# kirumang/Pix2Pose

Hardware: AMD Instinct MI355X
Metric: crops/sec (AE fwd + PnP-RANSAC) at 128x128 (higher is better)
Workload: dtype f16x3 (fp32 operands split into two f16 halves, 3 MFMAs per product block, fp32 accumulate)

## Files before the change

### include/p2p_mi355.h

```cpp
#ifndef P2P_MI355_H
#define P2P_MI355_H

#include <stdint.h>

#ifdef __cplusplus
extern "C" {
#endif

#define P2P_ABI_VERSION 12

#if defined(__GNUC__)
#define P2P_API __attribute__((visibility("default")))
#else
#define P2P_API
#endif

typedef enum {
    P2P_OK = 0,
    P2P_ERR_INVALID_ARG = -1,
    P2P_ERR_HIP = -2,
    P2P_ERR_WEIGHTS = -3,
    P2P_ERR_CAPACITY = -4,
    P2P_ERR_RANGE = -5
} p2p_status;
// ... 5 lines not shown
typedef struct p2p_ctx p2p_ctx;
typedef struct p2p_model p2p_model;

typedef struct {
    const char* name;
    const float* data;
    int64_t numel;
} p2p_tensor;

P2P_API int p2p_abi_version(void);
P2P_API int p2p_abi_sizeof(int which);
P2P_API const char* p2p_build_id(void);
P2P_API int p2p_aa_weights(int side, double* w);
P2P_API int p2p_debug_back_resize(p2p_ctx* ctx, const float* prob, const float* pred, const float* non_gray, int out_h, int out_w,
                                  double th_inlier, int generation, unsigned char* q, unsigned char* below, unsigned char* ng_out);
P2P_API const char* p2p_last_error(void);
P2P_API int p2p_device_count(int* count);

P2P_API int p2p_ctx_create(int device, int max_batch, p2p_ctx** out);
P2P_API void p2p_ctx_destroy(p2p_ctx* ctx);
P2P_API int p2p_ctx_synchronize(p2p_ctx* ctx);
P2P_API void* p2p_ctx_stream(p2p_ctx* ctx);

P2P_API int p2p_model_create(p2p_ctx* ctx, const p2p_tensor* tensors, int n_tensors, int backbone,
                     p2p_model** out);

typedef enum { P2P_PREC_F32 = 0, P2P_PREC_F16X3 = 1, P2P_PREC_AUTO = 2 } p2p_precision;
#define P2P_PREC_DEFAULT P2P_PREC_F16X3
P2P_API int p2p_model_create_ex(p2p_ctx* ctx, const p2p_tensor* tensors, int n_tensors, int backbone,
                        int precision, p2p_model** out);
// ... 296 lines not shown
```

### pix2pose_amd/_lib.py

```python
from __future__ import annotations

import ctypes as C
import os

_HERE = os.path.dirname(os.path.abspath(__file__))
LIB_PATH = os.environ.get("P2P_LIB", os.path.join(_HERE, "libp2p_mi355.so"))

P2P_OK = 0
ABI_VERSION = 12
MAX_RANSAC_ITERATIONS = 128
BACKBONE = {"paper": 0, "resnet50": 1}
PRECISION = {"f32": 0, "f16x3": 1, "auto": 2}
ERR_RANGE = -5
MEM_HOST, MEM_DEVICE = 0, 1
COMM_ID_BYTES = 128
POSE_ABSENT = -1
POSE_RANGE = -2
TICKET_NONE = -1


class P2PError(RuntimeError):
    pass


# ... 213 lines not shown
        except Exception as e:
            raise P2PError("libp2p_mi355.so is %s and could not be rebuilt: %s" % (reason, e))
        reason = _stale_reason(LIB_PATH)
        if reason is not None:
            raise P2PError("%s: %s after a rebuild" % (LIB_PATH, reason))
    _preload_torch_hip()
    try:
        L = C.CDLL(LIB_PATH)
    except OSError as e:
        raise P2PError("cannot load %s: %s (the HIP path is mandatory, there is no fallback)" % (LIB_PATH, e))
    vp, fp, ci = C.c_void_p, C.POINTER(C.c_float), C.c_int
    L.p2p_abi_version.restype = ci
    L.p2p_abi_sizeof.argtypes = [ci]
    L.p2p_build_id.restype = C.c_char_p
    L.p2p_aa_weights.argtypes = [ci, C.POINTER(C.c_double)]
    L.p2p_last_error.restype = C.c_char_p
    L.p2p_device_count.argtypes = [C.POINTER(ci)]
    L.p2p_ctx_create.argtypes = [ci, ci, C.POINTER(vp)]
    L.p2p_ctx_destroy.argtypes = [vp]
    L.p2p_ctx_destroy.restype = None
    L.p2p_ctx_synchronize.argtypes = [vp]
    L.p2p_ctx_stream.argtypes = [vp]
    L.p2p_ctx_stream.restype = vp
    L.p2p_model_create.argtypes = [vp, C.POINTER(Tensor), ci, ci, C.POINTER(vp)]
    L.p2p_model_create_ex.argtypes = [vp, C.POINTER(Tensor), ci, ci, ci, C.POINTER(vp)]
    L.p2p_model_destroy.argtypes = [vp]
    L.p2p_model_destroy.restype = None
    L.p2p_model_precision.argtypes = [vp]
    L.p2p_ctx_range_event.argtypes = [vp, C.POINTER(C.c_float)]
    L.p2p_ctx_set_winograd.argtypes = [vp, ci]
# ... 56 lines not shown
```

### pix2pose_amd/csrc/kernels.h

```cpp
#pragma once
#include <hip/hip_runtime.h>
#include <stdint.h>
#include <stdlib.h>

namespace p2p {

#ifdef P2P_DEV_SWITCHES
inline const char* dev_env(const char* name) { return getenv(name); }
#else
inline const char* dev_env(const char*) { return nullptr; }
#endif

struct Ctx;
extern thread_local Ctx* g_prof_ctx;
struct ProfScope {
    Ctx* ctx;
    hipStream_t s;
    int slot;
    double flops, bytes;
    hipEvent_t a = nullptr, b = nullptr;
    bool failed = false;
    ProfScope(Ctx* X, int slot_, hipStream_t st, double fl = 0.0, double by = 0.0) : ctx(X), s(st), slot(slot_), flops(fl), bytes(by) { if (ctx) open(); }
    ProfScope(int slot_, hipStream_t st) : ProfScope(g_prof_ctx, slot_, st) {}
    ~ProfScope() { if (ctx) (void)close(); }
// ... 89 lines not shown

int igemm_halo8_mode(const IgemmParams& p);
hipError_t launch_igemm_halo8(const IgemmParams& p, hipStream_t s);

bool igemm_halo_s2_supported(const IgemmParams& p);
hipError_t launch_igemm_halo_s2(const IgemmParams& p, hipStream_t s);

struct ResBlockGroup {
    const float* w2a;
    const float* w2b;
    const float* w2c;
    const float* ss;
    int sample0;
    int pad_;
    const float* w2b_frag;
};
struct ResBlockParams {
    const float* x;
    float* out;
    int N, H, W;
    unsigned x_bytes, wa_bytes, wb_bytes, wc_bytes;
    unsigned* range_acc;
    int n_groups;
    ResBlockGroup grp[IGEMM_MAX_GROUPS + 1];
};
bool resblock_supported(int F1, int H, int W);
int resblock_grid(int F1, int N, int H, int W);
hipError_t launch_resblock(const ResBlockParams& p, int F1, hipStream_t s);
hipError_t launch_resproj(const ResBlockParams& p, int F1, hipStream_t s);

struct WinoGroup {
// ... 131 lines not shown
```

### pix2pose_amd/csrc/model.hip

```cpp
#include "model.h"

#include <cmath>
#include <cstdarg>
#include <cstdio>
#include <cstring>
#include <thread>

namespace p2p {

static thread_local char g_err[512] = "";

void set_error(const char* fmt, ...)
{
    va_list ap;
    va_start(ap, fmt);
    vsnprintf(g_err, sizeof(g_err), fmt, ap);
    va_end(ap);
}
const char* get_error() { return g_err; }

constexpr double BN_EPS = 1e-3;
constexpr float LEAKY = 0.3f;

struct TensorMap {
// ... 604 lines not shown
        if ((rc = pack_wino3_s2(T, {"conv4_1", "conv4_2"}, 512, 256, M.L["conv4"]))) return rc;
        return build_decoder(T, M, 128, 128, 32);
    }
    if (M.backbone == P2P_BACKBONE_PAPER) {
        if ((rc = pack_conv_first(T, {"conv1_1", "conv1_2"}, 5, 64, M.L["conv1"]))) return rc;
        if ((rc = pack_conv(T, {"conv2_1", "conv2_2"}, 5, 128, 128, 1, true, M.L["conv2"]))) return rc;
        if ((rc = pack_conv(T, {"conv3_1", "conv3_2"}, 5, 256, 128, 1, true, M.L["conv3"]))) return rc;
        if ((rc = pack_conv(T, {"conv4_1", "conv4_2"}, 5, 256, 256, 1, true, M.L["conv4"]))) return rc;
        if ((rc = pack_wino3_s2(T, {"conv4_1", "conv4_2"}, 256, 256, M.L["conv4"]))) return rc;
        return build_decoder(T, M, 128, 128, 64);
    }
    set_error("unknown backbone %d", M.backbone);
    return P2P_ERR_INVALID_ARG;
}

static int pack_block_ss(Model& M)
{
    if (M.backbone != P2P_BACKBONE_RESNET50 || M.prec != PREC_F16X3) return P2P_OK;
    for (const char* nm : {"res2a", "res2b", "res2c", "res3a", "res3b", "res3c", "res3d"}) {
        const std::string n = nm;
        if (!M.L.count(n + "_2c") && !M.L.count(n + "_2c1")) continue;
        const ConvLayer &a = M.L.at(n + "_2a"), &b = M.L.at(n + "_2b"), &c = M.L.count(n + "_2c") ? M.L.at(n + "_2c") : M.L.at(n + "_2c1");
        const int F1 = a.Cout, C = c.Cout;
        float* d = nullptr;
        HIP_TRY(hipMalloc((void**)&d, (size_t)(4 * F1 + 2 * C) * sizeof(float)));
        M.block_ss[n] = d;
        if (!M.L.at(n + "_2b").w_frag) {
            ConvLayer& Lb = M.L.at(n + "_2b");
            const int K = Lb.K, KS = K / 32, NTL = Lb.Cout / 32;
            std::vector<float> host((size_t)round_up(Lb.Cout, 128) * K), frag((size_t)Lb.Cout * K);
            HIP_TRY(hipMemcpy(host.data(), Lb.w, host.size() * sizeof(float), hipMemcpyDeviceToHost));
            const uint16_t* sh = reinterpret_cast<const uint16_t*>(host.data());
            uint16_t* dh = reinterpret_cast<uint16_t*>(frag.data());
            for (int nt = 0; nt < NTL; ++nt)
                for (int ks = 0; ks < KS; ++ks)
                    for (int f = 0; f < 4; ++f)
                        for (int lane = 0; lane < 64; ++lane) {
                            const int row = nt * 32 + (lane & 31), kb = f >> 1, hf = f & 1;
                            const uint16_t* sp = sh + ((size_t)row * K + (size_t)ks * 32) * 2 + hf * 32 + kb * 16 + (lane >> 5) * 8;
                            uint16_t* dp = dh + ((((size_t)nt * KS + ks) * 4 + f) * 64 + lane) * 8;
                            for (int e = 0; e < 8; ++e) dp[e] = sp[e];
                        }
            int rcu = upload(frag, &Lb.w_frag);
            if (rcu) return rcu;
        }
        const float* src[6] = {a.scale, a.shift, b.scale, b.shift, c.scale, c.shift};
        const int len[6] = {F1, F1, F1, F1, C, C};
        size_t off = 0;
        for (int k = 0; k < 6; ++k) {
            HIP_TRY(hipMemcpy(d + off, src[k], (size_t)len[k] * sizeof(float), hipMemcpyDeviceToDevice));
            off += len[k];
        }
    }
    return P2P_OK;
}

constexpr size_t WINO_PARTIAL_FLOATS = (size_t)256 * 16 * 32 * 64;
static const struct { const char* name; size_t per_sample; } kBuffers[] = {
// ... 481 lines not shown
    const size_t xb = (size_t)N * H * H * Cin * sizeof(float), ob = (size_t)N * Ho * Ho * C * sizeof(float);
    if (xb >= 0xFFFFFFF0ull || ob >= 0xFFFFFFF0ull) { set_error("run_fused_block: tensor exceeds the 4 GB buffer-descriptor range (lower max_batch)"); return P2P_ERR_CAPACITY; }
    p.x_bytes = (unsigned)xb;
    p.wa_bytes = (unsigned)((size_t)round_up(a.Cout, 128) * a.K * sizeof(float));
    p.wb_bytes = (unsigned)((size_t)round_up(b.Cout, 128) * b.K * sizeof(float));
    p.wc_bytes = (unsigned)((size_t)round_up(c.Cout, 128) * c.K * sizeof(float));
    p.range_acc = X.range_cur;
    const int ng = pass_groups(X, "run_fused_block");
    if (ng < 0) return ng;
    if (ng) {
        const GroupCtx& G = *X.grp;
        for (int g = 0; g < ng; ++g) {
            const Model& Mg = *G.models[g];
            const ConvLayer* bg = group_layer(X, g, b, false);
            if (!bg || !Mg.block_ss.count(n)) return group_mismatch("run_fused_block");
            p.grp[g] = {Mg.L.at(a.name).w, bg->w, Mg.L.at(c.name).w, Mg.block_ss.at(n), G.start[g], 0, bg->w_frag};
        }
        p.grp[ng] = {nullptr, nullptr, nullptr, nullptr, G.start[ng], 0, nullptr};
        p.n_groups = ng;
    } else {
        p.grp[0] = {a.w, b.w, c.w, M.block_ss.at(n), 0, 0, b.w_frag};
        p.grp[1] = {nullptr, nullptr, nullptr, nullptr, N, 0, nullptr};
        p.n_groups = 1;
    }
    const double px = (double)N * Ho * Ho;
    return prof_launch(X, 9, 2.0 * px * ((double)Cin * f1 + 9.0 * f1 * f1 + (double)c.K * C),
                       4.0 * (px * Cin + px * C + (double)Cin * f1 + 9.0 * f1 * f1 + (double)c.K * C),
                       [&]() { return proj ? launch_resproj(p, f1, X.cur->stream) : launch_resblock(p, f1, X.cur->stream); });
}

static bool fused_proj_blocks() { static const bool on = dev_env("P2P_NO_FUSED_PROJ") == nullptr; return on; }

static int res_block(const Model& M, Ctx& X, const std::string& n, const float* in, int N, int H,
                     int Cin, int f1, int stride, bool shortcut, float* out)
{
    int rc;
    const int Ho = H / stride;
// ... 287 lines not shown
    case 3: return (int)sizeof(p2p_detection);
    case 4: return (int)sizeof(p2p_pose);
    case 5: return (int)sizeof(p2p_est_pose_opts);
    case 6: return (int)sizeof(p2p_kernel_stats);
    case 7: return (int)sizeof(p2p_refine_job);
    case 8: return (int)sizeof(p2p_depth_score);
    case 9: return (int)sizeof(p2p_icp_input);
    case 10: return (int)sizeof(p2p_icp_params);
    case 11: return (int)sizeof(p2p_icp_result);
    case 12: return (int)sizeof(p2p_refine_result);
    default: return -1;
    }
}
const char* p2p_last_error(void) { return get_error(); }

int p2p_device_count(int* count)
{
    if (!count) { set_error("p2p_device_count: null argument"); return P2P_ERR_INVALID_ARG; }
    HIP_TRY(hipGetDeviceCount(count));
    return P2P_OK;
}

int p2p_ctx_create(int device, int max_batch, p2p_ctx** out)
{
    if (!out || max_batch < 1) { set_error("p2p_ctx_create: bad arguments"); return P2P_ERR_INVALID_ARG; }
    *out = nullptr;
    int n = 0;
    HIP_TRY(hipGetDeviceCount(&n));
    if (device < 0 || device >= n) { set_error("p2p_ctx_create: device %d out of range (%d devices)", device, n); return P2P_ERR_INVALID_ARG; }
    HIP_TRY(hipSetDevice(device));
// ... 189 lines not shown
```

### pix2pose_amd/csrc/resblock.hip

```cpp
#include "device_common.h"

namespace p2p {

namespace {

constexpr int REC = 144;
constexpr int WREC = 128;

constexpr int cmax(int a, int b) { return a > b ? a : b; }

#ifdef P2P_RB_NO_WDIR
constexpr bool RB_WDIR = false;
#else
constexpr bool RB_WDIR = true;
#endif
#ifndef P2P_RB_DA64
#define P2P_RB_DA64 2
#endif
#ifndef P2P_RB_DA3A
#define P2P_RB_DA3A 2
#endif
#ifdef P2P_RB_NO_PIPE
constexpr bool RB_PIPE = false;
#else
constexpr bool RB_PIPE = true;
#endif
#ifdef P2P_RB_NO_DBUF
constexpr bool RB_DBUF = false;
#else
constexpr bool RB_DBUF = true;
#endif
template <int F1, int PY, int HPX, int DA, int DB, int KA, bool PRIV, int ABL = 0, int CIN = 4 * F1, int STRIDE = 1, bool PROJ = false, bool WDIR = RB_WDIR, bool DBUF = RB_DBUF, bool PIPE = RB_PIPE>
__global__ __launch_bounds__(256, 2) void resblock_kernel(const ResBlockParams p)
{
    constexpr int C = 4 * F1;
    constexpr int SA = CIN / 32;
    constexpr int SX = CIN / 32;
    static_assert(PROJ || (CIN == C && STRIDE == 1), "identity blocks keep their shape");
    constexpr int SB = F1 / 32;
    constexpr int NCH = C / 128;
    constexpr int HX0 = HPX == 18 ? 1 : 0;
    constexpr int HPY = PY + 2, NPA = HPY * HPX, MA = (NPA + 31) / 32;
    constexpr int PITCH = (HPX * REC + 255) / 256 * 256;
    constexpr int TSLICE = HPY * PITCH, T_BYTES = SB * TSLICE;
    constexpr int NPIX = PY * 16, MT = PY / 2;
    constexpr int T2SLICE = NPIX * REC, T2_BYTES = SB * T2SLICE;
    constexpr int XS_BYTES = MA * 32 * REC;
    constexpr int WA_BYTES = F1 * WREC;
    constexpr int WB_BYTES = PRIV ? 4 * 32 * WREC : F1 * WREC;
    constexpr int WC_BYTES = 2 * 128 * WREC;
    constexpr int NST = SB / 2;
    constexpr int TMC = 2, TNC = MT == 4 ? 2 : 1, WGMC = MT / TMC, WGNC = 4 / WGMC;
    constexpr int CLD = 128 + 4;
    constexpr int CS_BYTES = TMC * 32 * CLD * 4;
    constexpr int XC_BYTES = NPIX * REC;
    constexpr int NBUF = DBUF ? 2 : KA;
    static_assert(!DBUF || (KA == 1 && DA % 2 == 0), "double buffering: one K-step per stage, buffer parity = ring slot parity");
    constexpr int ZERO_OFF = cmax(cmax(NBUF * (XS_BYTES + WA_BYTES), T_BYTES + WB_BYTES),
                                  T2_BYTES + cmax(PROJ ? 128 * WREC + XC_BYTES : WC_BYTES, CS_BYTES));
    constexpr int SS_OFF = ZERO_OFF + 128, SS_FLOATS = 4 * F1 + 2 * C;
    constexpr int SMEM = SS_OFF + SS_FLOATS * 4;
    static_assert(SMEM <= 80 * 1024, "two workgroups per CU");
    static_assert(MA % (F1 == 64 ? 2 : 1) == 0 && (F1 == 64 || F1 == 128) && (PY == 8 || PY == 4), "shapes");
    __shared__ __attribute__((aligned(256))) char smem[SMEM];
    static_assert(SS_FLOATS % 4 == 0, "float4 copies");

    const int tid = threadIdx.x;
    const int lane = tid & 63, wave = __builtin_amdgcn_readfirstlane(tid >> 6);
    const int li = lane & 31, lk = lane >> 5;

    const int tiles_x = p.W / 16, tiles_y = p.H / PY;
    int t = xcd_first_tile(gridDim.x, blockIdx.x);
    const int x0 = (t % tiles_x) * 16; t /= tiles_x;
    const int y0 = (t % tiles_y) * PY;
    const int n = t / tiles_y;

    int g = 0;
    while (g + 1 < p.n_groups && p.grp[g + 1].sample0 <= n) ++g;
    const float* ss = reinterpret_cast<const float*>(smem + SS_OFF);
    for (int i = tid * 4; i < SS_FLOATS; i += 1024)
        *reinterpret_cast<f32x4*>(smem + SS_OFF + i * 4) = *reinterpret_cast<const f32x4*>(p.grp[g].ss + i);
    const __amdgpu_buffer_rsrc_t rs_x = __builtin_amdgcn_make_buffer_rsrc((void*)p.x, 0, p.x_bytes, 0x00020000);
    const __amdgpu_buffer_rsrc_t rs_wa = __builtin_amdgcn_make_buffer_rsrc((void*)p.grp[g].w2a, 0, p.wa_bytes, 0x00020000);
    const __amdgpu_buffer_rsrc_t rs_wb = __builtin_amdgcn_make_buffer_rsrc((void*)p.grp[g].w2b, 0, p.wb_bytes, 0x00020000);
    const __amdgpu_buffer_rsrc_t rs_wc = __builtin_amdgcn_make_buffer_rsrc((void*)p.grp[g].w2c, 0, p.wc_bytes, 0x00020000);

    if (tid < 8) *reinterpret_cast<f32x4*>(smem + ZERO_OFF + tid * 16) = f32x4{0.f, 0.f, 0.f, 0.f};

    const int lrow = tid >> 3, lseg = tid & 7;
    const int w_dst = lrow * WREC + ((lseg ^ ((lrow >> 1) & 7)) << 4);
    float amax = 0.f;

    f32x16 accA[3];
#pragma unroll
    for (int i = 0; i < 3; ++i)
#pragma unroll
        for (int r = 0; r < 16; ++r) accA[i][r] = 0.f;
    constexpr int WNA = F1 / 32 >= 4 ? 4 : F1 / 32, WMA = 4 / WNA;
    static_assert(MA == 3 * WMA, "three m-tiles per wave");
    const int ntA = wave % WNA, mt0A = (wave / WNA) * 3;
// ... 16 lines not shown
        unsigned wa_off[F1 / 32];
#pragma unroll
        for (int j = 0; j < F1 / 32; ++j) wa_off[j] = ((unsigned)(lrow + 32 * j) * (unsigned)CIN + (unsigned)lseg * 4u) * 4u;
        constexpr int NSTG = SA / KA;
        static_assert(SA % KA == 0 && NSTG % DA == 0, "ring depth divides the stages");
        f32x4 rx[DA][KA][MA], rw[DA][KA][F1 / 32];
        auto gload = [&](int stg, auto& qx, auto& qw) {
#pragma unroll
            for (int k2 = 0; k2 < KA; ++k2) {
                const int s = stg * KA + k2;
#pragma unroll
                for (int j = 0; j < MA; ++j)
                    qx[k2][j] = (ABL & 4) ? f32x4{1.f, 2.f, 3.f, 4.f}
                                          : __builtin_bit_cast(f32x4, __builtin_amdgcn_raw_buffer_load_b128(rs_x, x_off[j], s * 128, 0));
#pragma unroll
                for (int j = 0; j < F1 / 32; ++j) qw[k2][j] = __builtin_bit_cast(f32x4, __builtin_amdgcn_raw_buffer_load_b128(rs_wa, wa_off[j], s * 128, 0));
            }
        };
        auto lstore = [&](const auto& qx, const auto& qw, int buf = 0) {
#pragma unroll
            for (int k2 = 0; k2 < KA; ++k2) {
                const int b = DBUF ? buf : k2;
#pragma unroll
                for (int j = 0; j < MA; ++j) {
                    uint2 hi, lo;
                    split4(qx[k2][j], hi, lo);
                    *reinterpret_cast<uint2*>(Xs + b * XS_BYTES + x_dst[j]) = hi;
                    *reinterpret_cast<uint2*>(Xs + b * XS_BYTES + x_dst[j] + 64) = lo;
                }
#pragma unroll
                for (int j = 0; j < F1 / 32; ++j) *reinterpret_cast<f32x4*>(Was + b * WA_BYTES + w_dst + 32 * j * WREC) = qw[k2][j];
            }
        };
#pragma unroll
        for (int d = 0; d < DA; ++d) gload(d, rx[d], rw[d]);
        lstore(rx[0], rw[0]);
        __syncthreads();
        const char* Xf = Xs + (mt0A * 32 + li) * REC + lk * 16;
        const char* Wf = Was + (ntA * 32 + li) * WREC;
        int w_sw[2][2];
#pragma unroll
        for (int kb = 0; kb < 2; ++kb)
#pragma unroll
            for (int hf = 0; hf < 2; ++hf) w_sw[kb][hf] = ((kb * 2 + lk + 4 * hf) ^ ((li >> 1) & 7)) << 4;
        for (int g0 = 0; g0 < NSTG; g0 += DA) {
#pragma unroll
            for (int d = 0; d < DA; ++d) {
                const int stg = g0 + d;
                if (stg + DA < NSTG) gload(stg + DA, rx[d], rw[d]);
                if constexpr (PIPE && KA == 1 && ABL == 0) {
                    const int b = DBUF ? (d & 1) : 0;
                    f16x8 wf[2][2], xf[2][3][2];
#pragma unroll
                    for (int kb = 0; kb < 2; ++kb) {
                        wf[kb][0] = *reinterpret_cast<const f16x8*>(Wf + b * WA_BYTES + w_sw[kb][0]);
                        wf[kb][1] = *reinterpret_cast<const f16x8*>(Wf + b * WA_BYTES + w_sw[kb][1]);
#pragma unroll
                        for (int i = 0; i < 3; ++i) {
                            xf[kb][i][0] = *reinterpret_cast<const f16x8*>(Xf + b * XS_BYTES + i * 32 * REC + kb * 32);
                            xf[kb][i][1] = *reinterpret_cast<const f16x8*>(Xf + b * XS_BYTES + i * 32 * REC + kb * 32 + 64);
                        }
                    }
                    __builtin_amdgcn_sched_barrier(0);
                    if (DBUF && stg + 1 < NSTG) lstore(rx[(d + 1) % DA], rw[(d + 1) % DA], (d + 1) & 1);
#pragma unroll
                    for (int kb = 0; kb < 2; ++kb)
#pragma unroll
                        for (int i = 0; i < 3; ++i) {
                            accA[i] = __builtin_amdgcn_mfma_f32_32x32x16_f16(wf[kb][0], xf[kb][i][1], accA[i], 0, 0, 0);
                            accA[i] = __builtin_amdgcn_mfma_f32_32x32x16_f16(wf[kb][1], xf[kb][i][0], accA[i], 0, 0, 0);
                            accA[i] = __builtin_amdgcn_mfma_f32_32x32x16_f16(wf[kb][0], xf[kb][i][0], accA[i], 0, 0, 0);
                        }
                } else {
                if (DBUF && stg + 1 < NSTG) lstore(rx[(d + 1) % DA], rw[(d + 1) % DA], (d + 1) & 1);
#pragma unroll
                for (int k2 = 0; k2 < KA; ++k2)
#pragma unroll
                    for (int kb = 0; kb < 2; ++kb) {
                        const int b = DBUF ? (d & 1) : k2;
                        const f16x8 wh = *reinterpret_cast<const f16x8*>(Wf + b * WA_BYTES + w_sw[kb][0]);
                        const f16x8 wl = *reinterpret_cast<const f16x8*>(Wf + b * WA_BYTES + w_sw[kb][1]);
#pragma unroll
                        for (int i = 0; i < 3; ++i) {
                            const f16x8 xh = *reinterpret_cast<const f16x8*>(Xf + b * XS_BYTES + i * 32 * REC + kb * 32);
                            const f16x8 xl = *reinterpret_cast<const f16x8*>(Xf + b * XS_BYTES + i * 32 * REC + kb * 32 + 64);
                            if (ABL & 32) { accA[i][0] += (float)wh[0] + (float)wl[0] + (float)xh[0] + (float)xl[0]; continue; }
                            accA[i] = __builtin_amdgcn_mfma_f32_32x32x16_f16(wh, xl, accA[i], 0, 0, 0);
                            accA[i] = __builtin_amdgcn_mfma_f32_32x32x16_f16(wl, xh, accA[i], 0, 0, 0);
                            accA[i] = __builtin_amdgcn_mfma_f32_32x32x16_f16(wh, xh, accA[i], 0, 0, 0);
                        }
                    }
                }
                __syncthreads();
                if (!DBUF && stg + 1 < NSTG) {
                    lstore(rx[(d + 1) % DA], rw[(d + 1) % DA]);
                    __syncthreads();
// ... 203 lines not shown
    f32x4 rwc[2][4];
    auto wcload = [&](int q, int st) {
#pragma unroll
        for (int k2 = 0; k2 < (PROJ ? 1 : 2); ++k2)
#pragma unroll
            for (int j = 0; j < 4; ++j)
                rwc[k2][j] = __builtin_bit_cast(f32x4, __builtin_amdgcn_raw_buffer_load_b128(rs_wc, wc_off[j] + (unsigned)(q * 128 * K2C * 4), ((PROJ ? st : 2 * st) + k2) * 128, 0));
    };
    char* Wcs = smem + T2_BYTES;
    auto wcstore = [&]() {
#pragma unroll
        for (int k2 = 0; k2 < (PROJ ? 1 : 2); ++k2)
#pragma unroll
            for (int j = 0; j < 4; ++j) *reinterpret_cast<f32x4*>(Wcs + k2 * 128 * WREC + w_dst + 32 * j * WREC) = rwc[k2][j];
    };
    wcload(0, 0);

    {
        char* T2 = smem + ntB * T2SLICE;
#pragma unroll
        for (int i = 0; i < 2; ++i) {
            char* dst = T2 + ((mt0B + i) * 32 + li) * REC + lk * 8;
#pragma unroll
            for (int gq = 0; gq < 4; ++gq) {
                const int c = ntB * 32 + 8 * gq + 4 * lk;
                const f32x4 sc = *reinterpret_cast<const f32x4*>(ss + 2 * F1 + c);
                const f32x4 sh = *reinterpret_cast<const f32x4*>(ss + 3 * F1 + c);
                f32x4 v;
#pragma unroll
                for (int e = 0; e < 4; ++e) v[e] = relu_nan(fmaf(accB[i][4 * gq + e], sc[e], sh[e]));
                amax = range_note4(amax, v);
                uint2 hi, lo;
                split4(v, hi, lo);
                *reinterpret_cast<uint2*>(dst + gq * 16) = hi;
                *reinterpret_cast<uint2*>(dst + gq * 16 + 64) = lo;
            }
        }
    }
    wcstore();
    __syncthreads();

    if constexpr (PROJ) {
        constexpr int KC = SB + SX, NSTAGE = KC * NCH;
        const int wm = wave / WGNC, wn = wave % WGNC;
        char* Xcs = Wcs + 128 * WREC;
        const char* Bf = Wcs + (wn * TNC * 32 + li) * WREC;
        int w_sw[2][2];
#pragma unroll
        for (int kb = 0; kb < 2; ++kb)
#pragma unroll
            for (int hf = 0; hf < 2; ++hf) w_sw[kb][hf] = ((kb * 2 + lk + 4 * hf) ^ ((li >> 1) & 7)) << 4;
        constexpr int XP = NPIX * 8 / 256;
        unsigned xc_off[XP];
        int xc_dst[XP];
#pragma unroll
        for (int j = 0; j < XP; ++j) {
            const int idx = tid + 256 * j;
            const int t8 = idx >> 3, q = idx & 7;
            const int px = (t8 & ~7) | ((t8 & 1) << 2) | ((t8 >> 1) & 3);
            xc_off[j] = (((unsigned)(n * p.H * STRIDE + (y0 + (px >> 4)) * STRIDE) * (unsigned)(p.W * STRIDE) + (unsigned)((x0 + (px & 15)) * STRIDE)) * (unsigned)CIN + (unsigned)(q * 4)) * 4u;
// ... 21 lines not shown
#pragma unroll
                for (int j = 0; j < TNC; ++j)
#pragma unroll
                    for (int r = 0; r < 16; ++r) acc[q][i][j][r] = 0.f;
#pragma unroll 1
        for (int ks = 0; ks < KC; ++ks) {
            const char* Af = (ks < SB ? smem + ks * T2SLICE : Xcs) + (wm * TMC * 32 + li) * REC + lk * 16;
            f16x8 ah[2][TMC], al[2][TMC];
#pragma unroll
            for (int kb = 0; kb < 2; ++kb)
#pragma unroll
                for (int i = 0; i < TMC; ++i) {
                    ah[kb][i] = *reinterpret_cast<const f16x8*>(Af + i * 32 * REC + kb * 32);
                    al[kb][i] = *reinterpret_cast<const f16x8*>(Af + i * 32 * REC + kb * 32 + 64);
                }
#pragma unroll
            for (int q = 0; q < NCH; ++q) {
                const int stage = ks * NCH + q;
                const bool more = stage + 1 < NSTAGE;
                const bool next_ks = q + 1 == NCH;
                if (more) {
                    wcload(next_ks ? 0 : q + 1, next_ks ? ks + 1 : ks);
                    if (next_ks && ks + 1 >= SB) xcload(ks + 1 - SB);
                }
#pragma unroll
                for (int kb = 0; kb < 2; ++kb) {
                    f16x8 bh[TNC], bl[TNC];
#pragma unroll
                    for (int j = 0; j < TNC; ++j) {
                        bh[j] = *reinterpret_cast<const f16x8*>(Bf + j * 32 * WREC + w_sw[kb][0]);
// ... 67 lines not shown
            const unsigned orow = (unsigned)(p.W * C);
            auto rsload = [&](int h) {
#pragma unroll
                for (int it = 0; it < NIT; ++it)
                    rs[it] = (ABL & 1) ? f32x4{0.f, 0.f, 0.f, 0.f}
                                       : *reinterpret_cast<const f32x4*>(p.x + (obase + (unsigned)(4 * h + (it >> 1)) * orow + (unsigned)(8 * (it & 1) * C)));
            };
            rsload(0);
            f32x16 acc[TMC][TNC];
#pragma unroll
            for (int i = 0; i < TMC; ++i)
#pragma unroll
                for (int j = 0; j < TNC; ++j)
#pragma unroll
                    for (int r = 0; r < 16; ++r) acc[i][j][r] = 0.f;
            for (int st = 0; st < NST; ++st) {
                const bool more = st + 1 < NST || q + 1 < NCH;
                if (more) wcload(st + 1 < NST ? q : q + 1, st + 1 < NST ? st + 1 : 0);
                if constexpr (PIPE && ABL == 0) {
                    f16x8 fa[2][TMC][2], fb[2][TNC][2];
                    auto fread = [&](int u, f16x8 (&qa)[TMC][2], f16x8 (&qb)[TNC][2]) {
                        const int k2 = u >> 1, kb = u & 1;
#pragma unroll
                        for (int i = 0; i < TMC; ++i) {
                            qa[i][0] = *reinterpret_cast<const f16x8*>(Af + (2 * st + k2) * T2SLICE + i * 32 * REC + kb * 32);
                            qa[i][1] = *reinterpret_cast<const f16x8*>(Af + (2 * st + k2) * T2SLICE + i * 32 * REC + kb * 32 + 64);
                        }
#pragma unroll
                        for (int j = 0; j < TNC; ++j) {
                            qb[j][0] = *reinterpret_cast<const f16x8*>(Bf + k2 * 128 * WREC + j * 32 * WREC + w_sw[kb][0]);
// ... 70 lines not shown
                    for (int e = 0; e < 4; ++e) v[e] += rs[it][e];
#pragma unroll
                    for (int e = 0; e < 4; ++e) v[e] = relu_nan(v[e]);
                    amax = range_note4(amax, v);
                    o[it] = v;
                }
                if (h + 1 < WGMC) rsload(h + 1);
#pragma unroll
                for (int it = 0; it < NIT; ++it) {
                    const f32x4 v = o[it];
                    if (!(ABL & 2) || v[0] == 12345.678f)
                        *reinterpret_cast<f32x4*>(p.out + (obase + (unsigned)(4 * h + (it >> 1)) * orow + (unsigned)(8 * (it & 1) * C))) = v;
                }
                __syncthreads();
            }
            if (q + 1 < NCH) {
                wcstore();
                __syncthreads();
            }
        }
    }
    }
    range_commit(p.range_acc, amax);
}

}

bool resblock_supported(int F1, int H, int W)
{
    return (F1 == 64 && H % 8 == 0 && W % 16 == 0 && W > 16) || (F1 == 128 && H % 4 == 0 && W == 16);
}

int resblock_grid(int F1, int N, int H, int W) { return N * (H / (F1 == 64 ? 8 : 4)) * (W / 16); }

hipError_t launch_resproj(const ResBlockParams& p, int F1, hipStream_t s)
{
    if (!resblock_supported(F1, p.H, p.W)) return hipErrorInvalidValue;
    const int grid = resblock_grid(F1, p.N, p.H, p.W);
    if (F1 == 64) hipLaunchKernelGGL((resblock_kernel<64, 8, 18, 2, 3, 1, false, 0, 64, 1, true>), dim3(grid), dim3(256), 0, s, p);
    else hipLaunchKernelGGL((resblock_kernel<128, 4, 16, P2P_RB_DA3A, 4, 1, false, 0, 256, 2, true>), dim3(grid), dim3(256), 0, s, p);
    return hipGetLastError();
}

hipError_t launch_resblock(const ResBlockParams& p, int F1, hipStream_t s)
{
    if (!resblock_supported(F1, p.H, p.W)) return hipErrorInvalidValue;
    const int grid = resblock_grid(F1, p.N, p.H, p.W);
#define P2P_RB_LAUNCH(KA_, DA_, PRIV_, ABL_)                                                                                              \
    do {                                                                                                                                  \
        if (F1 == 64) hipLaunchKernelGGL((resblock_kernel<64, 8, 18, (DA_ == 4 ? P2P_RB_DA64 : DA_), 3, KA_, PRIV_, ABL_>), dim3(grid), dim3(256), 0, s, p);      \
        else hipLaunchKernelGGL((resblock_kernel<128, 4, 16, DA_, 4, KA_, PRIV_, ABL_>), dim3(grid), dim3(256), 0, s, p);              \
    } while (0)
#ifdef P2P_DEV_SWITCHES
    static const int variant = dev_env("P2P_RB_VARIANT") ? atoi(dev_env("P2P_RB_VARIANT")) : 1;
    static const int abl = dev_env("P2P_RB_ABL") ? atoi(dev_env("P2P_RB_ABL")) : 0;
    switch (abl) {
    case 1: P2P_RB_LAUNCH(1, 4, false, 1); return hipGetLastError();
    case 2: P2P_RB_LAUNCH(1, 4, false, 2); return hipGetLastError();
    case 3: P2P_RB_LAUNCH(1, 4, false, 3); return hipGetLastError();
    case 4: P2P_RB_LAUNCH(1, 4, false, 4); return hipGetLastError();
    case 7: P2P_RB_LAUNCH(1, 4, false, 7); return hipGetLastError();
    case 8: P2P_RB_LAUNCH(1, 4, false, 8); return hipGetLastError();
    case 16: P2P_RB_LAUNCH(1, 4, false, 16); return hipGetLastError();
    case 32: P2P_RB_LAUNCH(1, 4, false, 32); return hipGetLastError();
    case 48: P2P_RB_LAUNCH(1, 4, false, 48); return hipGetLastError();
    default: break;
// ... 13 lines not shown
```

Before: 12140.

## Load 2a and 2c resblock weights directly from fragment-ordered global buffers

Pre-permutes the 2a and 2c conv weights into per-lane MFMA fragment order on the host at model load, alongside the existing 2b permutation. Kernel variants can then read these fragments straight into registers with buffer loads, bypassing the LDS weight staging. This drops LDS traffic and the barriers that store the weights, and shrinks shared memory. Defaults turn this on for the F1=128 blocks (both 2a and 2c) and leave F1=64 off. The cost is more registers for prefetched fragments and repeated global or L2 reads of the weights by every workgroup.

```diff
diff --git a/include/p2p_mi355.h b/include/p2p_mi355.h
--- a/include/p2p_mi355.h
+++ b/include/p2p_mi355.h
@@ -43,6 +43,7 @@
 P2P_API int p2p_aa_weights(int side, double* w);
 P2P_API int p2p_debug_back_resize(p2p_ctx* ctx, const float* prob, const float* pred, const float* non_gray, int out_h, int out_w,
                                   double th_inlier, int generation, unsigned char* q, unsigned char* below, unsigned char* ng_out);
+P2P_API int p2p_debug_frag_order(const float* panel, int rows, int K, float* frag);
 P2P_API const char* p2p_last_error(void);
 P2P_API int p2p_device_count(int* count);
 
diff --git a/pix2pose_amd/_lib.py b/pix2pose_amd/_lib.py
--- a/pix2pose_amd/_lib.py
+++ b/pix2pose_amd/_lib.py
@@ -251,6 +251,7 @@
     L.p2p_abi_sizeof.argtypes = [ci]
     L.p2p_build_id.restype = C.c_char_p
     L.p2p_aa_weights.argtypes = [ci, C.POINTER(C.c_double)]
+    L.p2p_debug_frag_order.argtypes = [vp, ci, ci, vp]
     L.p2p_last_error.restype = C.c_char_p
     L.p2p_device_count.argtypes = [C.POINTER(ci)]
     L.p2p_ctx_create.argtypes = [ci, ci, C.POINTER(vp)]
diff --git a/pix2pose_amd/csrc/kernels.h b/pix2pose_amd/csrc/kernels.h
--- a/pix2pose_amd/csrc/kernels.h
+++ b/pix2pose_amd/csrc/kernels.h
@@ -127,7 +127,10 @@
     int sample0;
     int pad_;
     const float* w2b_frag;
-};
+    const float* w2a_frag;
+    const float* w2c_frag;
+};
+void frag_order(const uint16_t* panel, int rows, int K, uint16_t* frag);
 struct ResBlockParams {
     const float* x;
     float* out;
diff --git a/pix2pose_amd/csrc/model.hip b/pix2pose_amd/csrc/model.hip
--- a/pix2pose_amd/csrc/model.hip
+++ b/pix2pose_amd/csrc/model.hip
@@ -642,6 +642,20 @@
     return P2P_ERR_INVALID_ARG;
 }
 
+void frag_order(const uint16_t* sh, int rows, int K, uint16_t* dh)
+{
+    const int KS = K / 32, NTL = rows / 32;
+    for (int nt = 0; nt < NTL; ++nt)
+        for (int ks = 0; ks < KS; ++ks)
+            for (int f = 0; f < 4; ++f)
+                for (int lane = 0; lane < 64; ++lane) {
+                    const int row = nt * 32 + (lane & 31), kb = f >> 1, hf = f & 1;
+                    const uint16_t* sp = sh + ((size_t)row * K + (size_t)ks * 32) * 2 + hf * 32 + kb * 16 + (lane >> 5) * 8;
+                    uint16_t* dp = dh + ((((size_t)nt * KS + ks) * 4 + f) * 64 + lane) * 8;
+                    for (int e = 0; e < 8; ++e) dp[e] = sp[e];
+                }
+}
+
 static int pack_block_ss(Model& M)
 {
     if (M.backbone != P2P_BACKBONE_RESNET50 || M.prec != PREC_F16X3) return P2P_OK;
@@ -653,23 +667,13 @@
         float* d = nullptr;
         HIP_TRY(hipMalloc((void**)&d, (size_t)(4 * F1 + 2 * C) * sizeof(float)));
         M.block_ss[n] = d;
-        if (!M.L.at(n + "_2b").w_frag) {
-            ConvLayer& Lb = M.L.at(n + "_2b");
-            const int K = Lb.K, KS = K / 32, NTL = Lb.Cout / 32;
-            std::vector<float> host((size_t)round_up(Lb.Cout, 128) * K), frag((size_t)Lb.Cout * K);
-            HIP_TRY(hipMemcpy(host.data(), Lb.w, host.size() * sizeof(float), hipMemcpyDeviceToHost));
-            const uint16_t* sh = reinterpret_cast<const uint16_t*>(host.data());
-            uint16_t* dh = reinterpret_cast<uint16_t*>(frag.data());
-            for (int nt = 0; nt < NTL; ++nt)
-                for (int ks = 0; ks < KS; ++ks)
-                    for (int f = 0; f < 4; ++f)
-                        for (int lane = 0; lane < 64; ++lane) {
-                            const int row = nt * 32 + (lane & 31), kb = f >> 1, hf = f & 1;
-                            const uint16_t* sp = sh + ((size_t)row * K + (size_t)ks * 32) * 2 + hf * 32 + kb * 16 + (lane >> 5) * 8;
-                            uint16_t* dp = dh + ((((size_t)nt * KS + ks) * 4 + f) * 64 + lane) * 8;
-                            for (int e = 0; e < 8; ++e) dp[e] = sp[e];
-                        }
-            int rcu = upload(frag, &Lb.w_frag);
+        for (const std::string& ln : {n + "_2a", n + "_2b", n + (M.L.count(n + "_2c") ? "_2c" : "_2c1")}) {
+            ConvLayer& Lf = M.L.at(ln);
+            if (Lf.w_frag) continue;
+            std::vector<float> host((size_t)round_up(Lf.Cout, 128) * Lf.K), frag((size_t)Lf.Cout * Lf.K);
+            HIP_TRY(hipMemcpy(host.data(), Lf.w, host.size() * sizeof(float), hipMemcpyDeviceToHost));
+            frag_order(reinterpret_cast<const uint16_t*>(host.data()), Lf.Cout, Lf.K, reinterpret_cast<uint16_t*>(frag.data()));
+            int rcu = upload(frag, &Lf.w_frag);
             if (rcu) return rcu;
         }
         const float* src[6] = {a.scale, a.shift, b.scale, b.shift, c.scale, c.shift};
@@ -1181,13 +1185,13 @@
             const Model& Mg = *G.models[g];
             const ConvLayer* bg = group_layer(X, g, b, false);
             if (!bg || !Mg.block_ss.count(n)) return group_mismatch("run_fused_block");
-            p.grp[g] = {Mg.L.at(a.name).w, bg->w, Mg.L.at(c.name).w, Mg.block_ss.at(n), G.start[g], 0, bg->w_frag};
-        }
-        p.grp[ng] = {nullptr, nullptr, nullptr, nullptr, G.start[ng], 0, nullptr};
+            p.grp[g] = {Mg.L.at(a.name).w, bg->w, Mg.L.at(c.name).w, Mg.block_ss.at(n), G.start[g], 0, bg->w_frag, Mg.L.at(a.name).w_frag, Mg.L.at(c.name).w_frag};
+        }
+        p.grp[ng] = {nullptr, nullptr, nullptr, nullptr, G.start[ng], 0, nullptr, nullptr, nullptr};
         p.n_groups = ng;
     } else {
-        p.grp[0] = {a.w, b.w, c.w, M.block_ss.at(n), 0, 0, b.w_frag};
-        p.grp[1] = {nullptr, nullptr, nullptr, nullptr, N, 0, nullptr};
+        p.grp[0] = {a.w, b.w, c.w, M.block_ss.at(n), 0, 0, b.w_frag, a.w_frag, c.w_frag};
+        p.grp[1] = {nullptr, nullptr, nullptr, nullptr, N, 0, nullptr, nullptr, nullptr};
         p.n_groups = 1;
     }
     const double px = (double)N * Ho * Ho;
@@ -1505,6 +1509,13 @@
 }
 const char* p2p_last_error(void) { return get_error(); }
 
+int p2p_debug_frag_order(const float* panel, int rows, int K, float* frag)
+{
+    if (!panel || !frag || rows <= 0 || K <= 0 || rows % 32 || K % 32) { set_error("p2p_debug_frag_order: bad arguments"); return P2P_ERR_INVALID_ARG; }
+    frag_order(reinterpret_cast<const uint16_t*>(panel), rows, K, reinterpret_cast<uint16_t*>(frag));
+    return P2P_OK;
+}
+
 int p2p_device_count(int* count)
 {
     if (!count) { set_error("p2p_device_count: null argument"); return P2P_ERR_INVALID_ARG; }
diff --git a/pix2pose_amd/csrc/resblock.hip b/pix2pose_amd/csrc/resblock.hip
--- a/pix2pose_amd/csrc/resblock.hip
+++ b/pix2pose_amd/csrc/resblock.hip
@@ -30,7 +30,19 @@
 #else
 constexpr bool RB_DBUF = true;
 #endif
-template <int F1, int PY, int HPX, int DA, int DB, int KA, bool PRIV, int ABL = 0, int CIN = 4 * F1, int STRIDE = 1, bool PROJ = false, bool WDIR = RB_WDIR, bool DBUF = RB_DBUF, bool PIPE = RB_PIPE>
+#ifndef P2P_RB_WFRAG64
+#define P2P_RB_WFRAG64 0
+#endif
+#ifndef P2P_RB_WFRAG128
+#define P2P_RB_WFRAG128 3
+#endif
+#ifndef P2P_RB_WFRAG2A
+#define P2P_RB_WFRAG2A 0
+#endif
+#ifndef P2P_RB_WFRAG3A
+#define P2P_RB_WFRAG3A 3
+#endif
+template <int F1, int PY, int HPX, int DA, int DB, int KA, bool PRIV, int ABL = 0, int CIN = 4 * F1, int STRIDE = 1, bool PROJ = false, bool WDIR = RB_WDIR, bool DBUF = RB_DBUF, bool PIPE = RB_PIPE, bool CDIR = false, bool ADIR = false>
 __global__ __launch_bounds__(256, 2) void resblock_kernel(const ResBlockParams p)
 {
     constexpr int C = 4 * F1;
@@ -46,8 +58,8 @@
     constexpr int NPIX = PY * 16, MT = PY / 2;
     constexpr int T2SLICE = NPIX * REC, T2_BYTES = SB * T2SLICE;
     constexpr int XS_BYTES = MA * 32 * REC;
-    constexpr int WA_BYTES = F1 * WREC;
-    constexpr int WB_BYTES = PRIV ? 4 * 32 * WREC : F1 * WREC;
+    constexpr int WA_BYTES = ADIR ? 0 : F1 * WREC;
+    constexpr int WB_BYTES = WDIR ? 0 : PRIV ? 4 * 32 * WREC : F1 * WREC;
     constexpr int WC_BYTES = 2 * 128 * WREC;
     constexpr int NST = SB / 2;
     constexpr int TMC = 2, TNC = MT == 4 ? 2 : 1, WGMC = MT / TMC, WGNC = 4 / WGMC;
@@ -57,7 +69,9 @@
     constexpr int NBUF = DBUF ? 2 : KA;
     static_assert(!DBUF || (KA == 1 && DA % 2 == 0), "double buffering: one K-step per stage, buffer parity = ring slot parity");
     constexpr int ZERO_OFF = cmax(cmax(NBUF * (XS_BYTES + WA_BYTES), T_BYTES + WB_BYTES),
-                                  T2_BYTES + cmax(PROJ ? 128 * WREC + XC_BYTES : WC_BYTES, CS_BYTES));
+                                  T2_BYTES + cmax(PROJ ? (CDIR ? 0 : 128 * WREC) + XC_BYTES : (CDIR ? 0 : WC_BYTES), CS_BYTES));
+    static_assert(!ADIR || KA == 1, "direct 2a weights: one K-step per stage");
+    static_assert(!CDIR || (PIPE && ABL == 0), "direct 2c weights: the pipelined form only");
     constexpr int SS_OFF = ZERO_OFF + 128, SS_FLOATS = 4 * F1 + 2 * C;
     constexpr int SMEM = SS_OFF + SS_FLOATS * 4;
     static_assert(SMEM <= 80 * 1024, "two workgroups per CU");
@@ -84,6 +98,8 @@
     const __amdgpu_buffer_rsrc_t rs_wa = __builtin_amdgcn_make_buffer_rsrc((void*)p.grp[g].w2a, 0, p.wa_bytes, 0x00020000);
     const __amdgpu_buffer_rsrc_t rs_wb = __builtin_amdgcn_make_buffer_rsrc((void*)p.grp[g].w2b, 0, p.wb_bytes, 0x00020000);
     const __amdgpu_buffer_rsrc_t rs_wc = __builtin_amdgcn_make_buffer_rsrc((void*)p.grp[g].w2c, 0, p.wc_bytes, 0x00020000);
+    const __amdgpu_buffer_rsrc_t rs_waf = __builtin_amdgcn_make_buffer_rsrc((void*)p.grp[g].w2a_frag, 0, (unsigned)(F1 * CIN * 4), 0x00020000);
+    const __amdgpu_buffer_rsrc_t rs_wcf = __builtin_amdgcn_make_buffer_rsrc((void*)p.grp[g].w2c_frag, 0, (unsigned)(C * (PROJ ? F1 + CIN : F1) * 4), 0x00020000);
 
     if (tid < 8) *reinterpret_cast<f32x4*>(smem + ZERO_OFF + tid * 16) = f32x4{0.f, 0.f, 0.f, 0.f};
 
@@ -130,7 +146,8 @@
                     qx[k2][j] = (ABL & 4) ? f32x4{1.f, 2.f, 3.f, 4.f}
                                           : __builtin_bit_cast(f32x4, __builtin_amdgcn_raw_buffer_load_b128(rs_x, x_off[j], s * 128, 0));
 #pragma unroll
-                for (int j = 0; j < F1 / 32; ++j) qw[k2][j] = __builtin_bit_cast(f32x4, __builtin_amdgcn_raw_buffer_load_b128(rs_wa, wa_off[j], s * 128, 0));
+                for (int j = 0; j < F1 / 32; ++j)
+                    if (!ADIR) qw[k2][j] = __builtin_bit_cast(f32x4, __builtin_amdgcn_raw_buffer_load_b128(rs_wa, wa_off[j], s * 128, 0));
             }
         };
         auto lstore = [&](const auto& qx, const auto& qw, int buf = 0) {
@@ -145,11 +162,21 @@
                     *reinterpret_cast<uint2*>(Xs + b * XS_BYTES + x_dst[j] + 64) = lo;
                 }
 #pragma unroll
-                for (int j = 0; j < F1 / 32; ++j) *reinterpret_cast<f32x4*>(Was + b * WA_BYTES + w_dst + 32 * j * WREC) = qw[k2][j];
+                for (int j = 0; j < F1 / 32; ++j)
+                    if (!ADIR) *reinterpret_cast<f32x4*>(Was + b * WA_BYTES + w_dst + 32 * j * WREC) = qw[k2][j];
             }
         };
-#pragma unroll
-        for (int d = 0; d < DA; ++d) gload(d, rx[d], rw[d]);
+        f16x8 raf[DA][4];
+        auto afload = [&](int s, f16x8 (&q)[4]) {
+            const unsigned base = (unsigned)((ntA * SA + s) * 4096);
+#pragma unroll
+            for (int f = 0; f < 4; ++f) q[f] = __builtin_bit_cast(f16x8, __builtin_amdgcn_raw_buffer_load_b128(rs_waf, (unsigned)lane * 16u + f * 1024u, base, 0));
+        };
+#pragma unroll
+        for (int d = 0; d < DA; ++d) {
+            gload(d, rx[d], rw[d]);
+            if (ADIR) afload(d, raf[d]);
+        }
         lstore(rx[0], rw[0]);
         __syncthreads();
         const char* Xf = Xs + (mt0A * 32 + li) * REC + lk * 16;
@@ -163,14 +190,25 @@
 #pragma unroll
             for (int d = 0; d < DA; ++d) {
                 const int stg = g0 + d;
-                if (stg + DA < NSTG) gload(stg + DA, rx[d], rw[d]);
+                f16x8 wq[4];
+                if (ADIR) {
+#pragma unroll
+                    for (int f = 0; f < 4; ++f) wq[f] = raf[d][f];
+                }
+                if (stg + DA < NSTG) {
+                    gload(stg + DA, rx[d], rw[d]);
+                    if (ADIR) afload(stg + DA, raf[d]);
+                }
                 if constexpr (PIPE && KA == 1 && ABL == 0) {
                     const int b = DBUF ? (d & 1) : 0;
                     f16x8 wf[2][2], xf[2][3][2];
 #pragma unroll
                     for (int kb = 0; kb < 2; ++kb) {
-                        wf[kb][0] = *reinterpret_cast<const f16x8*>(Wf + b * WA_BYTES + w_sw[kb][0]);
-                        wf[kb][1] = *reinterpret_cast<const f16x8*>(Wf + b * WA_BYTES + w_sw[kb][1]);
+                        if (ADIR) { wf[kb][0] = wq[2 * kb]; wf[kb][1] = wq[2 * kb + 1]; }
+                        else {
+                            wf[kb][0] = *reinterpret_cast<const f16x8*>(Wf + b * WA_BYTES + w_sw[kb][0]);
+                            wf[kb][1] = *reinterpret_cast<const f16x8*>(Wf + b * WA_BYTES + w_sw[kb][1]);
+                        }
 #pragma unroll
                         for (int i = 0; i < 3; ++i) {
                             xf[kb][i][0] = *reinterpret_cast<const f16x8*>(Xf + b * XS_BYTES + i * 32 * REC + kb * 32);
@@ -194,8 +232,8 @@
 #pragma unroll
                     for (int kb = 0; kb < 2; ++kb) {
                         const int b = DBUF ? (d & 1) : k2;
-                        const f16x8 wh = *reinterpret_cast<const f16x8*>(Wf + b * WA_BYTES + w_sw[kb][0]);
-                        const f16x8 wl = *reinterpret_cast<const f16x8*>(Wf + b * WA_BYTES + w_sw[kb][1]);
+                        const f16x8 wh = ADIR ? wq[2 * kb] : *reinterpret_cast<const f16x8*>(Wf + b * WA_BYTES + w_sw[kb][0]);
+                        const f16x8 wl = ADIR ? wq[2 * kb + 1] : *reinterpret_cast<const f16x8*>(Wf + b * WA_BYTES + w_sw[kb][1]);
 #pragma unroll
                         for (int i = 0; i < 3; ++i) {
                             const f16x8 xh = *reinterpret_cast<const f16x8*>(Xf + b * XS_BYTES + i * 32 * REC + kb * 32);
@@ -429,7 +467,23 @@
 #pragma unroll
             for (int j = 0; j < 4; ++j) *reinterpret_cast<f32x4*>(Wcs + k2 * 128 * WREC + w_dst + 32 * j * WREC) = rwc[k2][j];
     };
-    wcload(0, 0);
+    constexpr int DC = 2, KSC = K2C / 32, NSTEP_C = NCH * (PROJ ? SB + SX : SB);
+    constexpr bool RCOPY = PROJ || TNC == 1;
+    const int wnC = wave % WGNC;
+    f16x8 rcf[DC][TNC][4];
+    auto cfload = [&](int step, f16x8 (&r)[TNC][4]) {
+        const int q = PROJ ? step % NCH : step / SB, ks = PROJ ? step / NCH : step % SB;
+#pragma unroll
+        for (int j = 0; j < TNC; ++j) {
+            const unsigned base = (unsigned)(((q * 4 + wnC * TNC + j) * KSC + ks) * 4096);
+#pragma unroll
+            for (int f = 0; f < 4; ++f) r[j][f] = __builtin_bit_cast(f16x8, __builtin_amdgcn_raw_buffer_load_b128(rs_wcf, (unsigned)lane * 16u + f * 1024u, base, 0));
+        }
+    };
+    if constexpr (CDIR) {
+#pragma unroll
+        for (int d = 0; d < (RCOPY ? DC : 1); ++d) cfload(d, rcf[d]);
+    } else wcload(0, 0);
 
     {
         char* T2 = smem + ntB * T2SLICE;
@@ -452,13 +506,13 @@
             }
         }
     }
-    wcstore();
+    if constexpr (!CDIR) wcstore();
     __syncthreads();
 
     if constexpr (PROJ) {
         constexpr int KC = SB + SX, NSTAGE = KC * NCH;
         const int wm = wave / WGNC, wn = wave % WGNC;
-        char* Xcs = Wcs + 128 * WREC;
+        char* Xcs = Wcs + (CDIR ? 0 : 128 * WREC);
         const char* Bf = Wcs + (wn * TNC * 32 + li) * WREC;
         int w_sw[2][2];
 #pragma unroll
@@ -510,6 +564,36 @@
                     ah[kb][i] = *reinterpret_cast<const f16x8*>(Af + i * 32 * REC + kb * 32);
                     al[kb][i] = *reinterpret_cast<const f16x8*>(Af + i * 32 * REC + kb * 32 + 64);
                 }
+            if constexpr (CDIR) {
+#pragma unroll
+                for (int q = 0; q < NCH; ++q) {
+                    const int stage = ks * NCH + q;
+                    f16x8 wq[TNC][4];
+#pragma unroll
+                    for (int j = 0; j < TNC; ++j)
+#pragma unroll
+                        for (int f = 0; f < 4; ++f) wq[j][f] = rcf[q % DC][j][f];
+                    if (stage + DC < NSTAGE) cfload(stage + DC, rcf[q % DC]);
+                    if (q == 0 && ks + 1 < KC && ks + 1 >= SB) xcload(ks + 1 - SB);
+                    __builtin_amdgcn_sched_barrier(0);
+#pragma unroll
+                    for (int kb = 0; kb < 2; ++kb)
+#pragma unroll
+                        for (int i = 0; i < TMC; ++i)
+#pragma unroll
+                            for (int j = 0; j < TNC; ++j) {
+                                acc[q][i][j] = __builtin_amdgcn_mfma_f32_32x32x16_f16(al[kb][i], wq[j][2 * kb], acc[q][i][j], 0, 0, 0);
+                                acc[q][i][j] = __builtin_amdgcn_mfma_f32_32x32x16_f16(ah[kb][i], wq[j][2 * kb + 1], acc[q][i][j], 0, 0, 0);
+                                acc[q][i][j] = __builtin_amdgcn_mfma_f32_32x32x16_f16(ah[kb][i], wq[j][2 * kb], acc[q][i][j], 0, 0, 0);
+                            }
+                    __builtin_amdgcn_sched_barrier(0);
+                }
+                if (ks + 1 < KC && ks + 1 >= SB) {
+                    __syncthreads();
+                    xcstore();
+                    __syncthreads();
+                } else if (ks + 1 == KC) __syncthreads();
+            } else
 #pragma unroll
             for (int q = 0; q < NCH; ++q) {
                 const int stage = ks * NCH + q;
@@ -607,6 +691,42 @@
                 for (int j = 0; j < TNC; ++j)
 #pragma unroll
                     for (int r = 0; r < 16; ++r) acc[i][j][r] = 0.f;
+            if constexpr (CDIR) {
+                f16x8 fa[2][TMC][2], wq[TNC][4];
+                auto aread = [&](int u, f16x8 (&qa)[TMC][2]) {
+                    const int ks = u >> 1, kb = u & 1;
+#pragma unroll
+                    for (int i = 0; i < TMC; ++i) {
+                        qa[i][0] = *reinterpret_cast<const f16x8*>(Af + ks * T2SLICE + i * 32 * REC + kb * 32);
+                        qa[i][1] = *reinterpret_cast<const f16x8*>(Af + ks * T2SLICE + i * 32 * REC + kb * 32 + 64);
+                    }
+                };
+                aread(0, fa[0]);
+#pragma unroll
+                for (int u = 0; u < 2 * SB; ++u) {
+                    const int ks = u >> 1, kb = u & 1;
+                    if (kb == 0 && RCOPY) {
+#pragma unroll
+                        for (int j = 0; j < TNC; ++j)
+#pragma unroll
+                            for (int f = 0; f < 4; ++f) wq[j][f] = rcf[ks % DC][j][f];
+                        if (q * SB + ks + DC < NSTEP_C) cfload(q * SB + ks + DC, rcf[ks % DC]);
+                    }
+                    if (kb == 0 && !RCOPY && q * SB + ks + 1 < NSTEP_C) cfload(q * SB + ks + 1, rcf[(ks + 1) % DC]);
+                    if (u + 1 < 2 * SB) aread(u + 1, fa[(u + 1) & 1]);
+                    __builtin_amdgcn_sched_barrier(0);
+#pragma unroll
+                    for (int i = 0; i < TMC; ++i)
+#pragma unroll
+                        for (int j = 0; j < TNC; ++j) {
+                            const f16x8 bh = RCOPY ? wq[j][2 * kb] : rcf[ks % DC][j][2 * kb], bl = RCOPY ? wq[j][2 * kb + 1] : rcf[ks % DC][j][2 * kb + 1];
+                            acc[i][j] = __builtin_amdgcn_mfma_f32_32x32x16_f16(fa[u & 1][i][1], bh, acc[i][j], 0, 0, 0);
+                            acc[i][j] = __builtin_amdgcn_mfma_f32_32x32x16_f16(fa[u & 1][i][0], bl, acc[i][j], 0, 0, 0);
+                            acc[i][j] = __builtin_amdgcn_mfma_f32_32x32x16_f16(fa[u & 1][i][0], bh, acc[i][j], 0, 0, 0);
+                        }
+                    __builtin_amdgcn_sched_barrier(0);
+                }
+            } else
             for (int st = 0; st < NST; ++st) {
                 const bool more = st + 1 < NST || q + 1 < NCH;
                 if (more) wcload(st + 1 < NST ? q : q + 1, st + 1 < NST ? st + 1 : 0);
@@ -707,7 +827,7 @@
                 }
                 __syncthreads();
             }
-            if (q + 1 < NCH) {
+            if (!CDIR && q + 1 < NCH) {
                 wcstore();
                 __syncthreads();
             }
@@ -730,8 +850,8 @@
 {
     if (!resblock_supported(F1, p.H, p.W)) return hipErrorInvalidValue;
     const int grid = resblock_grid(F1, p.N, p.H, p.W);
-    if (F1 == 64) hipLaunchKernelGGL((resblock_kernel<64, 8, 18, 2, 3, 1, false, 0, 64, 1, true>), dim3(grid), dim3(256), 0, s, p);
-    else hipLaunchKernelGGL((resblock_kernel<128, 4, 16, P2P_RB_DA3A, 4, 1, false, 0, 256, 2, true>), dim3(grid), dim3(256), 0, s, p);
+    if (F1 == 64) hipLaunchKernelGGL((resblock_kernel<64, 8, 18, 2, 3, 1, false, 0, 64, 1, true, RB_WDIR, RB_DBUF, RB_PIPE, RB_PIPE && (P2P_RB_WFRAG2A & 1), (P2P_RB_WFRAG2A & 2) != 0>), dim3(grid), dim3(256), 0, s, p);
+    else hipLaunchKernelGGL((resblock_kernel<128, 4, 16, P2P_RB_DA3A, 4, 1, false, 0, 256, 2, true, RB_WDIR, RB_DBUF, RB_PIPE, RB_PIPE && (P2P_RB_WFRAG3A & 1), (P2P_RB_WFRAG3A & 2) != 0>), dim3(grid), dim3(256), 0, s, p);
     return hipGetLastError();
 }
 
@@ -741,8 +861,8 @@
     const int grid = resblock_grid(F1, p.N, p.H, p.W);
 #define P2P_RB_LAUNCH(KA_, DA_, PRIV_, ABL_)                                                                                              \
     do {                                                                                                                                  \
-        if (F1 == 64) hipLaunchKernelGGL((resblock_kernel<64, 8, 18, (DA_ == 4 ? P2P_RB_DA64 : DA_), 3, KA_, PRIV_, ABL_>), dim3(grid), dim3(256), 0, s, p);      \
-        else hipLaunchKernelGGL((resblock_kernel<128, 4, 16, DA_, 4, KA_, PRIV_, ABL_>), dim3(grid), dim3(256), 0, s, p);              \
+        if (F1 == 64) hipLaunchKernelGGL((resblock_kernel<64, 8, 18, (DA_ == 4 ? P2P_RB_DA64 : DA_), 3, KA_, PRIV_, ABL_, 256, 1, false, RB_WDIR, RB_DBUF, RB_PIPE, RB_PIPE && ABL_ == 0 && (P2P_RB_WFRAG64 & 1), ABL_ == 0 && (P2P_RB_WFRAG64 & 2)>), dim3(grid), dim3(256), 0, s, p);      \
+        else hipLaunchKernelGGL((resblock_kernel<128, 4, 16, DA_, 4, KA_, PRIV_, ABL_, 512, 1, false, RB_WDIR, RB_DBUF, RB_PIPE, RB_PIPE && ABL_ == 0 && (P2P_RB_WFRAG128 & 1), ABL_ == 0 && (P2P_RB_WFRAG128 & 2)>), dim3(grid), dim3(256), 0, s, p);              \
     } while (0)
 #ifdef P2P_DEV_SWITCHES
     static const int variant = dev_env("P2P_RB_VARIANT") ? atoi(dev_env("P2P_RB_VARIANT")) : 1;
```

Measured after the change: 12220 (median of 6 runs). No clear change (+0.7%).
